# helenypzhang/Subspace-Multimodal-Learning

Hardware: AMD Instinct MI355X
Metric: bags/sec fwd+bwd, DeformCrossTransMIL N=10k x 512 (higher is better)
Workload: dtype f32

## Files before the change

subspace-multimodal-learning_amd/csrc/deform_attn.hip:

```cpp
#include "deform_common.h"
#include "cpb_regions.h"
#include "cpb_regions1d.h"

extern "C" int smml_deform_attn_nst(int N);

namespace {


constexpr int FWD_WPS = 2;
template <int PDX, bool SAVE>
__global__ __launch_bounds__(256, FWD_WPS) void deform_attn_fwd_kernel(
    const float* __restrict__ Q, const float* __restrict__ K, const float* __restrict__ V,
    const float* __restrict__ VS, const float* __restrict__ GQ, CpbParams cp, float* __restrict__ O,
    float* __restrict__ LSE, float* __restrict__ LT, unsigned short* __restrict__ MK, int N, int J, int H, int G, int NST,
    float scale, DropCfg dc_in) {
  constexpr int PD = PosCfg<PDX>::PD;
  constexpr bool RAW = PosCfg<PDX>::RAW;
  const DropCfg dc = drop_resolve(dc_in);
  __shared__ __attribute__((aligned(16))) _Float16 Kp[2][KT * FRLD];
  __shared__ __attribute__((aligned(16))) _Float16 Vp[2][KT * FTLD];
  __shared__ __attribute__((aligned(16))) _Float16 Qp[WAVES][2][QT * FRLD];
  __shared__ float vsl[KT][2];
  __shared__ float biasT[WAVES][KT][QT];

// ... 133 lines not shown
    wave_lds_fence();

    float tmax = -INFINITY;
#pragma unroll
    for (int r = 0; r < 16; ++r) {
      const int key = acc_row(r, hf);
      const float sv = (key < nk) ? s[r] + biasT[wave][key][c] : -INFINITY;
      s[r] = sv;
      tmax = fmaxf(tmax, sv);
    }
    unsigned keepbits = 0xFFFFu;
    if (dc.thresh) {
      const unsigned long long base2 = ((unsigned long long)(b * H + h) * N + qi) * ((J + 1) >> 1) + (j0 >> 1);
      keepbits = 0u;
#pragma unroll
      for (int r = 0; r < 16; r += 2) keepbits |= drop_keep2(dc, base2 + (acc_row(r, hf) >> 1)) << r;
    }
    if (SAVE) {
      if (dc.thresh) {
        tmax = -INFINITY;
#pragma unroll
        for (int r = 0; r < 16; ++r) {
          if (acc_row(r, hf) < nk) s[r] = stash_keep(s[r], (keepbits >> r) & 1u);
          tmax = fmaxf(tmax, s[r]);
        }
      }
#pragma unroll
      for (int r = 0; r < 16; ++r) {
        const int key = acc_row(r, hf);
        if (key < nk) LTb[(size_t)(j0 + key) * 32 + c] = s[r];
      }
    }
    tmax = xhalf_max(tmax);
    const float m_new = fmaxf(m_run, tmax);
    const float alpha = sexp(m_run - m_new);
    float psum = 0.f;
#pragma unroll
    for (int r = 0; r < 16; ++r) {
      const float p = sexp(s[r] - m_new);
      psum += p;
      s[r] = p;
    }
    if (dc.thresh) {
#pragma unroll
      for (int r = 0; r < 16; ++r) s[r] *= ((keepbits >> r) & 1u) ? dc.keep_scale : 0.f;
    }
    l_run = l_run * alpha + psum;
    m_run = m_new;
#pragma unroll
    for (int r = 0; r < 16; ++r) { oacc0[r] *= alpha; oacc1[r] *= alpha; }

#pragma unroll
    for (int kb = 0; kb < 2; ++kb) {
      float p8[8];
#pragma unroll
      for (int j = 0; j < 8; ++j) p8[j] = s[8 * kb + j];
      half8 ph, pl;
      split8(p8, ph, pl);
      const int ro = (16 * kb + 4 * hf + trq) * FTLD + trc;
      const half8 vh0 = lds_frag_tr_h(&Vp[0][ro], &Vp[0][ro + 8 * FTLD]), vl0 = lds_frag_tr_h(&Vp[1][ro], &Vp[1][ro + 8 * FTLD]);
      const half8 vh1 = lds_frag_tr_h(&Vp[0][ro + 32], &Vp[0][ro + 32 + 8 * FTLD]), vl1 = lds_frag_tr_h(&Vp[1][ro + 32], &Vp[1][ro + 32 + 8 * FTLD]);
      oacc0 = mfma16(vl0, ph, oacc0); oacc0 = mfma16(vh0, pl, oacc0); oacc0 = mfma16(vh0, ph, oacc0);
      oacc1 = mfma16(vl1, ph, oacc1); oacc1 = mfma16(vh1, pl, oacc1); oacc1 = mfma16(vh1, ph, oacc1);
    }
    wave_lds_fence();
  }

  l_run = xhalf_sum(l_run);
  const float inv = 1.f / l_run;
  if (qvalid) {
    float* op = O + ((size_t)b * N + qi) * HD + h * DH;
#pragma unroll
    for (int rg = 0; rg < 4; ++rg) {
      const int d = 8 * rg + 4 * hf;
      *reinterpret_cast<float4*>(op + d) = make_float4(oacc0[4 * rg] * inv, oacc0[4 * rg + 1] * inv,
                                                       oacc0[4 * rg + 2] * inv, oacc0[4 * rg + 3] * inv);
      *reinterpret_cast<float4*>(op + 32 + d) = make_float4(oacc1[4 * rg] * inv, oacc1[4 * rg + 1] * inv,
                                                            oacc1[4 * rg + 2] * inv, oacc1[4 * rg + 3] * inv);
    }
    if (hf == 0) LSE[(size_t)(b * H + h) * N + qi] = m_run + logf(l_run);
  }
}


__global__ __launch_bounds__(256, 2) void deform_attn_bwd_dq_kernel(
    const float* __restrict__ K, const float* __restrict__ V, const float* __restrict__ O,
    const float* __restrict__ dO, const float* __restrict__ LSE, const float* __restrict__ LT,
    float* __restrict__ dLT, float* __restrict__ dQ, float* __restrict__ RHO, unsigned* __restrict__ AMAX, int N, int J, int H, int NST,
    float scale, DropCfg dc_in) {
  const DropCfg dc = drop_resolve(dc_in);
  __shared__ __attribute__((aligned(16))) __bf16 Vp[2][3][KT * VBLD];
  __shared__ __attribute__((aligned(16))) __bf16 Kp[2][3][KT * KBLD];

  const int tid = threadIdx.x, wave = tid >> 6, lane = tid & 63, c = lane & 31, hf = lane >> 5;
  const int b = blockIdx.z, h = blockIdx.y;
  const int q0 = blockIdx.x * (QT * WAVES) + wave * QT;
  const int HD = H * DH;
  const bool qvalid = (q0 + c) < N;
  const int qi = qvalid ? (q0 + c) : (N - 1);

  bf16x8 doh[4], dom[4], dol[4];
  float delta = 0.f;
  {
    const size_t off = ((size_t)b * N + qi) * HD + h * DH + hf * 8;
#pragma unroll
    for (int kb = 0; kb < 4; ++kb) {
      const float4 t0 = *reinterpret_cast<const float4*>(dO + off + 16 * kb), t1 = *reinterpret_cast<const float4*>(dO + off + 16 * kb + 4);
      const float4 u0 = *reinterpret_cast<const float4*>(O + off + 16 * kb), u1 = *reinterpret_cast<const float4*>(O + off + 16 * kb + 4);
      delta += t0.x * u0.x + t0.y * u0.y + t0.z * u0.z + t0.w * u0.w + t1.x * u1.x + t1.y * u1.y + t1.z * u1.z + t1.w * u1.w;
      const float x8[8] = {t0.x, t0.y, t0.z, t0.w, t1.x, t1.y, t1.z, t1.w};
      split8_bf3(x8, doh[kb], dom[kb], dol[kb]);
    }
  }
  delta = xhalf_sum(delta);
  const float nl = prob_bias(LSE[(size_t)(b * H + h) * N + qi]);

  floatx16 dq0 = {0}, dq1 = {0};
  float amax = 0.f;
  float rho = 0.f;
  const float* Kb = K + (size_t)b * J * HD + h * DH;
  const float* Vb = V + (size_t)b * J * HD + h * DH;
  const float* LTb = LT + ((size_t)(b * H + h) * NST + q0) * J;
  float* dLTb = dLT + ((size_t)(b * H + h) * NST + q0) * J;

  const int skey = tid >> 4, sd4 = (tid & 15) * 4;
  const int trq = (lane & 15) >> 2, trc = 16 * ((lane >> 4) & 1) + 4 * (lane & 3);
  float4 kreg[2], vreg[2];
  float lt[16];
  auto fetch = [&](int j0, float4 (&kr)[2], float4 (&vr)[2], float (&l)[16]) {
#pragma unroll
    for (int i = 0; i < 2; ++i) {
      const int key = j0 + skey + 16 * i;
      kr[i] = make_float4(0.f, 0.f, 0.f, 0.f); vr[i] = kr[i];
      if (key < J) {
        kr[i] = *reinterpret_cast<const float4*>(Kb + (size_t)key * HD + sd4);
        vr[i] = *reinterpret_cast<const float4*>(Vb + (size_t)key * HD + sd4);
      }
    }
#pragma unroll
    for (int r = 0; r < 16; ++r) {
      const int key = min(j0 + acc_row(r, hf), J - 1);
      l[r] = LTb[(size_t)key * 32 + c];
    }
  };
  fetch(0, kreg, vreg, lt);

  const int ntiles = (J + KT - 1) / KT;
  for (int kt = 0; kt < ntiles; ++kt) {
    const int j0 = kt * KT, buf = kt & 1;
    const int nk = min(KT, J - j0);
#pragma unroll
    for (int i = 0; i < 2; ++i) {
      const int key = skey + 16 * i;
      uint2v hh, mm, ll;
      split4_bf3(vreg[i], hh, mm, ll);
      *reinterpret_cast<uint2v*>(&Vp[buf][0][key * VBLD + sd4]) = hh;
      *reinterpret_cast<uint2v*>(&Vp[buf][1][key * VBLD + sd4]) = mm;
      *reinterpret_cast<uint2v*>(&Vp[buf][2][key * VBLD + sd4]) = ll;
      split4_bf3(kreg[i], hh, mm, ll);
      *reinterpret_cast<uint2v*>(&Kp[buf][0][key * KBLD + sd4]) = hh;
      *reinterpret_cast<uint2v*>(&Kp[buf][1][key * KBLD + sd4]) = mm;
    }
    __syncthreads();
    float ltc[16];
#pragma unroll
    for (int r = 0; r < 16; ++r) ltc[r] = lt[r];
    if (kt + 1 < ntiles) fetch(j0 + KT, kreg, vreg, lt);

    floatx16 dp = {0};
#pragma unroll
    for (int kb = 0; kb < 4; ++kb) {
      const int o = c * VBLD + 16 * kb + 8 * hf;
      const bf16x8 vh = *reinterpret_cast<const bf16x8*>(&Vp[buf][0][o]);
      const bf16x8 vm = *reinterpret_cast<const bf16x8*>(&Vp[buf][1][o]);
      const bf16x8 vl = *reinterpret_cast<const bf16x8*>(&Vp[buf][2][o]);
      dp = bwd_prod<3>(vh, vm, vl, doh[kb], dom[kb], dol[kb], dp);
    }

    float ds[16];
    if (nk == KT && q0 + QT <= N) {
#pragma unroll
      for (int r = 0; r < 16; ++r) {
        const float p = prob_of(ltc[r], nl);
        float dpr = dp[r];
        if (dc.thresh) dpr *= stashed_factor(ltc[r], dc.keep_scale);
        const float v = p * (dpr - delta);
        dLTb[(size_t)(j0 + acc_row(r, hf)) * 32 + c] = v;
        ds[r] = v;
        rho += v;
        amax = fmaxf(amax, fabsf(v));
      }
    } else {
#pragma unroll
      for (int r = 0; r < 16; ++r) {
        const int key = acc_row(r, hf);
        float v = 0.f;
        if (key < nk && qvalid) {
          const float p = prob_of(ltc[r], nl);
          float dpr = dp[r];
          if (dc.thresh) dpr *= stashed_factor(ltc[r], dc.keep_scale);
          v = p * (dpr - delta);
          dLTb[(size_t)(j0 + key) * 32 + c] = v;
        }
        ds[r] = v;
        rho += v;
        amax = fmaxf(amax, fabsf(v));
      }
    }
#pragma unroll
    for (int kb = 0; kb < 2; ++kb) {
      float x8[8];
#pragma unroll
      for (int jx = 0; jx < 8; ++jx) x8[jx] = ds[8 * kb + jx];
      bf16x8 sh, sm, sl;
      split8_bf3(x8, sh, sm, sl);
      const int ro = (16 * kb + 4 * hf + trq) * KBLD + trc;
#pragma unroll
      for (int db = 0; db < 2; ++db) {
        const bf16x8 kh = lds_frag_tr(&Kp[buf][0][ro + 32 * db], &Kp[buf][0][ro + 32 * db + 8 * KBLD]);
        const bf16x8 km = lds_frag_tr(&Kp[buf][1][ro + 32 * db], &Kp[buf][1][ro + 32 * db + 8 * KBLD]);
        if (db == 0) dq0 = bwd_prod<2>(kh, km, km, sh, sm, sm, dq0);
        else dq1 = bwd_prod<2>(kh, km, km, sh, sm, sm, dq1);
      }
    }
  }
  rho = xhalf_sum(rho);
  if (qvalid && hf == 0) RHO[(size_t)(b * H + h) * N + qi] = rho;
  if (AMAX) {
    amax = wave_max_all(amax);
    if (lane == 0 && amax > 0.f) atomicMax(AMAX, __float_as_uint(amax));
  }
  if (qvalid) {
    float* qp = dQ + ((size_t)b * N + qi) * HD + h * DH;
#pragma unroll
    for (int rg = 0; rg < 4; ++rg) {
      const int d = 8 * rg + 4 * hf;
      *reinterpret_cast<float4*>(qp + d) = make_float4(dq0[4 * rg] * scale, dq0[4 * rg + 1] * scale,
                                                       dq0[4 * rg + 2] * scale, dq0[4 * rg + 3] * scale);
      *reinterpret_cast<float4*>(qp + 32 + d) = make_float4(dq1[4 * rg] * scale, dq1[4 * rg + 1] * scale,
                                                            dq1[4 * rg + 2] * scale, dq1[4 * rg + 3] * scale);
    }
  }
}


__global__ __launch_bounds__(256, 2) void deform_attn_bwd_dkv_kernel(
    const float* __restrict__ Q, const float* __restrict__ dO, const float* __restrict__ LSE,
    const float* __restrict__ LT, const float* __restrict__ dLT, float* __restrict__ dKp,
    float* __restrict__ dVp, int N, int J, int H, int NST, int nkg, int tiles_per_part, int nparts, int Bn, DropCfg dc_in) {
  const DropCfg dc = drop_resolve(dc_in);
  __shared__ __attribute__((aligned(16))) __bf16 Qp[2][3][QT * QBLD];
  __shared__ __attribute__((aligned(16))) __bf16 dOp[2][3][QT * QBLD];
  __shared__ __attribute__((aligned(16))) float nls[2][QT];
  const int tid = threadIdx.x, wave = tid >> 6, lane = tid & 63, c = lane & 31, hf = lane >> 5;
  const int nslices = nparts * H * Bn;
  const int chunk = blockIdx.x / (8 * nkg), rem = blockIdx.x - chunk * (8 * nkg);
  const int kg = rem >> 3, slice = chunk * 8 + (rem & 7);
  if (slice >= nslices) return;
  const int part = slice % nparts, h = (slice / nparts) % H, b = slice / (nparts * H);
  const int j0 = kg * DKV_KEYS + wave * KT;
  const int HD = H * DH;
  const int nk = min(KT, J - j0);
  const bool kvalid = c < nk;
  const int key = min(j0 + c, J - 1);
  const float* LTk = LT + (size_t)(b * H + h) * NST * J + (size_t)key * 32;
  const float* dLTk = dLT + (size_t)(b * H + h) * NST * J + (size_t)key * 32;
  const float* LSEb = LSE + (size_t)(b * H + h) * N;

  const int nqt = (N + QT - 1) / QT;
  const int qt_begin = part * tiles_per_part, qt_end = min(qt_begin + tiles_per_part, nqt);

  const int srow = tid >> 4, sd4 = (tid & 15) * 4;
  const int trq = (lane & 15) >> 2, trc = 16 * ((lane >> 4) & 1) + 4 * (lane & 3);
  float4 qreg[2], doreg[2], ltr[4], dlr[4];
  float lsereg = 0.f;
#pragma unroll
  for (int i = 0; i < 4; ++i) { ltr[i] = make_float4(0.f, 0.f, 0.f, 0.f); dlr[i] = ltr[i]; qreg[i >> 1] = ltr[i]; doreg[i >> 1] = ltr[i]; }
  auto fetch = [&](int q0) {
#pragma unroll
    for (int i = 0; i < 2; ++i) {
      const int qrow = min(q0 + srow + 16 * i, N - 1);
      const size_t off = ((size_t)b * N + qrow) * HD + h * DH + sd4;
      qreg[i] = *reinterpret_cast<const float4*>(Q + off);
      doreg[i] = *reinterpret_cast<const float4*>(dO + off);
    }
#pragma unroll
    for (int rg = 0; rg < 4; ++rg) {
      const size_t qq = (size_t)q0 * J + 8 * rg + 4 * hf;
      ltr[rg] = *reinterpret_cast<const float4*>(LTk + qq);
      dlr[rg] = *reinterpret_cast<const float4*>(dLTk + qq);
    }
    if (tid < QT) lsereg = LSEb[min(q0 + tid, N - 1)];
  };

  floatx16 dk0 = {0}, dk1 = {0}, dv0 = {0}, dv1 = {0};
  if (qt_begin < qt_end) fetch(qt_begin * QT);
  for (int qt = qt_begin; qt < qt_end; ++qt) {
    const int q0 = qt * QT, buf = (qt - qt_begin) & 1;
#pragma unroll
    for (int i = 0; i < 2; ++i) {
      const int o = (srow + 16 * i) * QBLD + sd4;
      uint2v hh, mm, ll;
      split4_bf3(qreg[i], hh, mm, ll);
      *reinterpret_cast<uint2v*>(&Qp[buf][0][o]) = hh;
      *reinterpret_cast<uint2v*>(&Qp[buf][1][o]) = mm;
      split4_bf3(doreg[i], hh, mm, ll);
      *reinterpret_cast<uint2v*>(&dOp[buf][0][o]) = hh;
      *reinterpret_cast<uint2v*>(&dOp[buf][1][o]) = mm;
    }
    if (tid < QT) nls[buf][tid] = prob_bias(lsereg);
    __syncthreads();
    float lv[16], dsv[16], ls[16];
#pragma unroll
    for (int rg = 0; rg < 4; ++rg) {
      lv[4 * rg + 0] = ltr[rg].x; lv[4 * rg + 1] = ltr[rg].y; lv[4 * rg + 2] = ltr[rg].z; lv[4 * rg + 3] = ltr[rg].w;
      dsv[4 * rg + 0] = dlr[rg].x; dsv[4 * rg + 1] = dlr[rg].y; dsv[4 * rg + 2] = dlr[rg].z; dsv[4 * rg + 3] = dlr[rg].w;
      const float4 t = *reinterpret_cast<const float4*>(&nls[buf][8 * rg + 4 * hf]);
      ls[4 * rg + 0] = t.x; ls[4 * rg + 1] = t.y; ls[4 * rg + 2] = t.z; ls[4 * rg + 3] = t.w;
    }
    if (qt + 1 < qt_end) fetch(q0 + QT);
    if (nk > 0) {
      float p[16], ds[16];
      if (nk == KT && q0 + QT <= N) {
#pragma unroll
        for (int r = 0; r < 16; ++r) {
          float pv = prob_of(lv[r], ls[r]);
          if (dc.thresh) pv *= stashed_factor(lv[r], dc.keep_scale);
          p[r] = pv; ds[r] = dsv[r];
        }
      } else {
#pragma unroll
        for (int r = 0; r < 16; ++r) {
          const int qq = q0 + acc_row(r, hf);
          const bool ok = kvalid && qq < N;
          float pv = ok ? prob_of(lv[r], ls[r]) : 0.f;
          if (dc.thresh && ok) pv *= stashed_factor(lv[r], dc.keep_scale);
          p[r] = pv;
          ds[r] = ok ? dsv[r] : 0.f;
        }
      }
#pragma unroll
      for (int kb = 0; kb < 2; ++kb) {
        float x8[8], y8[8];
#pragma unroll
        for (int jx = 0; jx < 8; ++jx) { x8[jx] = p[8 * kb + jx]; y8[jx] = ds[8 * kb + jx]; }
        bf16x8 ph, pm, pl, sh, sm, sl;
        split8_bf3(x8, ph, pm, pl);
        split8_bf3(y8, sh, sm, sl);
        const int ro = (16 * kb + 4 * hf + trq) * QBLD + trc;
#pragma unroll
        for (int db = 0; db < 2; ++db) {
          const int o = ro + 32 * db;
          const bf16x8 ah = lds_frag_tr(&dOp[buf][0][o], &dOp[buf][0][o + 8 * QBLD]);
          const bf16x8 am = lds_frag_tr(&dOp[buf][1][o], &dOp[buf][1][o + 8 * QBLD]);
          const bf16x8 qh = lds_frag_tr(&Qp[buf][0][o], &Qp[buf][0][o + 8 * QBLD]);
          const bf16x8 qm = lds_frag_tr(&Qp[buf][1][o], &Qp[buf][1][o + 8 * QBLD]);
          if (db == 0) { dv0 = bwd_prod<2>(ah, am, am, ph, pm, pm, dv0); dk0 = bwd_prod<2>(qh, qm, qm, sh, sm, sm, dk0); }
          else { dv1 = bwd_prod<2>(ah, am, am, ph, pm, pm, dv1); dk1 = bwd_prod<2>(qh, qm, qm, sh, sm, sm, dk1); }
        }
      }
    }
  }
  if (kvalid) {
    const size_t off = (((size_t)part * Bn + b) * J + (j0 + c)) * HD + h * DH;
    float* kp = dKp + off;
    float* vp = dVp + off;
#pragma unroll
    for (int rg = 0; rg < 4; ++rg) {
      const int d = 8 * rg + 4 * hf;
      *reinterpret_cast<float4*>(kp + d) = make_float4(dk0[4 * rg], dk0[4 * rg + 1], dk0[4 * rg + 2], dk0[4 * rg + 3]);
      *reinterpret_cast<float4*>(kp + 32 + d) = make_float4(dk1[4 * rg], dk1[4 * rg + 1], dk1[4 * rg + 2], dk1[4 * rg + 3]);
      *reinterpret_cast<float4*>(vp + d) = make_float4(dv0[4 * rg], dv0[4 * rg + 1], dv0[4 * rg + 2], dv0[4 * rg + 3]);
      *reinterpret_cast<float4*>(vp + 32 + d) = make_float4(dv1[4 * rg], dv1[4 * rg + 1], dv1[4 * rg + 2], dv1[4 * rg + 3]);
    }
  }
}


template <int PDX>
__global__ __launch_bounds__(256, 2) void cpb_bwd_kernel(
    const float* __restrict__ dLT, const unsigned short* __restrict__ MK, const float* __restrict__ LT,
    const float* __restrict__ LSE, const float* __restrict__ RHO, const float* __restrict__ VS,
    const float* __restrict__ GQ, CpbParams cp, float* __restrict__ slab, float* __restrict__ dvs_slab, int N, int J, int H,
    int G, int NST) {
  constexpr int PD = PosCfg<PDX>::PD;
  constexpr bool RAW = PosCfg<PDX>::RAW;
  extern __shared__ __attribute__((aligned(16))) float smem[];
  const int tid = threadIdx.x, wave = tid >> 6, lane = tid & 63, c = lane & 31, hf = lane >> 5;
  const int b = blockIdx.z, h = blockIdx.y;
  const int q0 = blockIdx.x * (QT * WAVES) + wave * QT;
  const int o = H / G, g = h / o, oi = h - g * o;
  const bool qvalid = (q0 + c) < N;
  const int qi = qvalid ? (q0 + c) : (N - 1);

  float* tab = smem;
  float* wbase = smem + CPB2_TAB;
  float* xq = wbase + wave * CPB2_WAVE_LDS;
  float2* stg = reinterpret_cast<float2*>(xq + CPB_XQ);
  const int wg = (blockIdx.z * gridDim.y + blockIdx.y) * gridDim.x + blockIdx.x;
  float2* dvs_row = reinterpret_cast<float2*>(dvs_slab) + (size_t)(wg * WAVES + wave) * J;
  if (tid < 32) {
    const int ch = acc_row(tid & 15, tid >> 4);
    tab[(tid >> 4) * 32 + (tid & 15)] = cp.w1[ch * PD];
    tab[(tid >> 4) * 32 + 16 + (tid & 15)] = (PD == 2) ? cp.w1[ch * PD + 1] : 0.f;
  }
  const float* tabh = tab + hf * 32;

  const float gq0 = GQ[(size_t)qi * PD];
  const float gq1 = (PD == 2) ? GQ[(size_t)qi * PD + 1] : 0.f;

  bf16x8 a1q, a1t;
  floatx16 b1acc;
  {
    const float wx = cp.w1[c * PD], wy = (PD == 2) ? cp.w1[c * PD + 1] : 0.f, bb = cp.b1[c];
    const __bf16 xh = (__bf16)wx; const float xr = wx - (float)xh; const __bf16 xm = (__bf16)xr;
    const __bf16 xl = (__bf16)(xr - (float)xm);
    const __bf16 yh = (__bf16)wy; const float yr = wy - (float)yh; const __bf16 ym = (__bf16)yr;
    const __bf16 yl = (__bf16)(yr - (float)ym);
    const __bf16 bh_ = (__bf16)bb; const float br = bb - (float)bh_; const __bf16 bm = (__bf16)br;
    const __bf16 bl_ = (__bf16)(br - (float)bm);
    const __bf16 z = (__bf16)0.f;
    a1q = cpb_l1_weights_q(wx, wy, hf);
    if (hf == 0) a1t = (bf16x8){xh, yh, xh, yh, xh, yh, bh_, bm};
    else a1t = (bf16x8){xm, ym, xm, ym, xl, yl, bl_, z};
#pragma unroll
    for (int s16 = 0; s16 < 16; ++s16) b1acc[s16] = cp.b1[acc_row(s16, hf)];
  }
  const float b2c = cp.b2[c];
  const float w3c = cp.w3[oi * CH + c];

  half8 w2th[2], w2tm[2], w2tl[2];
  half8 idb[2];
  float unlift2;
  {
    float amax = 0.f;
#pragma unroll
    for (int s = 0; s < 16; ++s) { const int ch = acc_row(s, hf); amax = fmaxf(amax, fabsf(cp.w2[ch * CH + c] * cp.w3[oi * CH + ch])); }
    const float lift2 = pow2_lift(wave_max_all(amax), 256.f, -8.f, 24.f);
    unlift2 = 1.f / lift2;
#pragma unroll
    for (int kb = 0; kb < 2; ++kb) {
      float t[8];
#pragma unroll
      for (int j = 0; j < 8; ++j) {
        const int ch = acc_row(8 * kb + j, hf);
        const float sc = (j & 1) ? 0.5f : 128.f;
        t[j] = cp.w2[ch * CH + c] * cp.w3[oi * CH + ch] * sc * lift2;
        idb[kb][j] = (ch == c) ? (_Float16)sc : (_Float16)0.0f;
      }
      split8_3(t, w2th[kb], w2tm[kb], w2tl[kb]);
    }
  }

  float big;
  asm("s_mov_b32 %0, 0x71800000" : "=s"(big));
  floatx16 e = {0};
  float2v aw1x[8], aw1y[8], ab1[8];
#pragma unroll
  for (int p = 0; p < 8; ++p) { aw1x[p] = (float2v){0.f, 0.f}; aw1y[p] = aw1x[p]; ab1[p] = aw1x[p]; }
  float ab3 = 0.f;
  float2v s2 = {0.f, 0.f};

  const float* VSb = VS + (size_t)(b * G + g) * J * PD;
  const float* dLTb = dLT + ((size_t)(b * H + h) * NST + q0) * J;
  __syncthreads();
// ... 147 lines not shown
    }
  }
#pragma unroll
  for (int r = 0; r < 16; ++r) {
    const int row = acc_row(r, hf);
    red[row * CH + c] = 0.5f * e[r] * cp.w3[oi * CH + row];
    float v;
    v = 0.5f * e[r] * cp.w2[row * CH + c];
#pragma unroll
    for (int off = 16; off > 0; off >>= 1) v += __shfl_xor(v, off);
    if (c == 0) red[1024 + 64 + 32 + 32 + row] += v;
    v = ab1[r >> 1][r & 1];
#pragma unroll
    for (int off = 16; off > 0; off >>= 1) v += __shfl_xor(v, off);
    if (c == 0) red[1024 + 64 + row] = v;
    v = aw1x[r >> 1][r & 1];
#pragma unroll
    for (int off = 16; off > 0; off >>= 1) v += __shfl_xor(v, off);
    if (c == 0) red[1024 + row * 2] = v;
    v = aw1y[r >> 1][r & 1];
#pragma unroll
    for (int off = 16; off > 0; off >>= 1) v += __shfl_xor(v, off);
    if (c == 0) red[1024 + row * 2 + 1] = v;
  }
  {
    float v = wave_sum(ab3);
    if (lane == 0) red[1024 + 64 + 32 + 32 + 32] = v;
  }
  __syncthreads();
  float* sl = slab + (size_t)wg * CPB_SLAB;
  const float* r0 = wbase + WAVES * CPB2_WAVE_LDS;
  for (int i = tid; i < CPB_SLAB; i += 256)
    sl[i] = (r0[i] + r0[CPB_SLAB + i]) + (r0[2 * CPB_SLAB + i] + r0[3 * CPB_SLAB + i]);
}


template <int PDX>
__global__ __launch_bounds__(256) void relu1_masks_kernel(const float* __restrict__ VS, const float* __restrict__ GQ,
                                                          const float* __restrict__ w1, const float* __restrict__ b1,
                                                          unsigned short* __restrict__ MK, int N, int J, int G, int NST) {
  constexpr int PD = PosCfg<PDX>::PD;
  constexpr bool RAW = PosCfg<PDX>::RAW;
  const int tid = threadIdx.x, wave = tid >> 6, lane = tid & 63, c = lane & 31, hf = lane >> 5;
  const int b = blockIdx.z, g = blockIdx.y;
  const int q0 = blockIdx.x * (QT * WAVES) + wave * QT;
  const int qi = min(q0 + c, N - 1);
  const float gq0 = GQ[(size_t)qi * PD];
  const float gq1 = (PD == 2) ? GQ[(size_t)qi * PD + 1] : 0.f;
  const bf16x8 a1 = cpb_l1_weights_q(w1[c * PD], (PD == 2) ? w1[c * PD + 1] : 0.f, hf);
  floatx16 b1acc;
#pragma unroll
  for (int s = 0; s < 16; ++s) b1acc[s] = b1[acc_row(s, hf)];
  const float* VSb = VS + (size_t)(b * G + g) * J * PD;
  unsigned short* MKb = MK + ((size_t)(b * G + g) * J * 2 + hf) * NST;
  for (int j = 0; j < J; ++j) {
    const float p0 = pos_of<RAW>(gq0 - VSb[(size_t)j * PD]);
    const float p1 = (PD == 2) ? slog1p(gq1 - VSb[(size_t)j * PD + 1]) : 0.f;
    const floatx16 xacc = cpb_layer1_q(a1, cpb_split_pos(p0, p1), hf, b1acc);
    unsigned m = 0;
#pragma unroll
    for (int r = 0; r < 16; ++r) m |= (xacc[r] > 0.f) ? (1u << ((13 + r) & 15)) : 0u;
    MKb[(size_t)j * 2 * NST + q0 + c] = (unsigned short)m;
  }
}


__global__ void drop_mask_kernel(float* __restrict__ mask, unsigned long long total, int J, DropCfg dc_in) {
  const DropCfg dc = drop_resolve(dc_in);
  const unsigned long long i = (unsigned long long)blockIdx.x * blockDim.x + threadIdx.x;
  if (i >= total) return;
  const unsigned long long row = i / (unsigned long long)J;
  const int j = (int)(i - row * (unsigned long long)J);
  mask[i] = (dc.thresh == 0 || ((drop_keep2(dc, row * (unsigned long long)((J + 1) >> 1) + (j >> 1)) >> (j & 1)) & 1u)) ? 1.f : 0.f;
}

template <int PDX> auto fwd_kernel(bool save) { return save ? deform_attn_fwd_kernel<PDX, true> : deform_attn_fwd_kernel<PDX, false>; }

int bwd_dq_dkv(const char* fn, const float* q, const float* k, const float* v, const float* out, const float* dout, const float* lse,
                      const float* logits_t, float* dlogits_t, float* dq, float* dk, float* dv, float* wsf, unsigned* amax, int B, int N, int J,
                      int H, float scale, DropCfg dc, hipStream_t st) {
  const BwdWorkspace wsl = bwd_workspace(B, N, J, H);
  const int nst = smml_deform_attn_nst(N);
  const int qtiles = (N + QT * WAVES - 1) / (QT * WAVES);
  hipLaunchKernelGGL(deform_attn_bwd_dq_kernel, dim3(qtiles, H, B), dim3(256), 0, st, k, v, out, dout, lse, logits_t, dlogits_t, dq, wsf + wsl.rho,
                     amax, N, J, H, nst, scale, dc);
  if (int rc = launch_check(fn, "dq")) return rc;
  const DkvGrid g = dkv_grid(B, N, J, H);
  hipLaunchKernelGGL(deform_attn_bwd_dkv_kernel, g.grid, dim3(256), 0, st, q, dout, lse, logits_t, dlogits_t, wsf + wsl.dkp, wsf + wsl.dvp, N, J, H,
                     nst, g.nkg, g.tpp, g.parts, B, dc);
  if (int rc = launch_check(fn, "dkv")) return rc;
  return dkv_reduce_launch(fn, wsf, wsl, dk, dv, B, J, H, g.parts, scale, st);
}

}

extern "C" {

int smml_deform_attn_nst(int N) { return (N <= 0 || N > SMML_MAX_QUERIES) ? 0 : (N + QT * WAVES - 1) / (QT * WAVES) * (QT * WAVES); }

int smml_deform_attn_dropout_mask_f32(float* mask, int B, int N, int J, int H, float dropout_p, unsigned long long dropout_seed,
                                      void* stream, const SmmlDeformOpts* opts) {
  SMML_REQUIRE(mask && deform_dims_ok(B, N, J, H) && dropout_p >= 0.f && dropout_p < 1.f,
               "smml_deform_attn_dropout_mask_f32: bad argument");
  const unsigned long long total = (unsigned long long)B * H * N * J;
  hipLaunchKernelGGL(drop_mask_kernel, dim3((unsigned)((total + 255) / 256)), dim3(256), 0, (hipStream_t)stream, mask, total, J,
                     make_drop(dropout_p, dropout_seed, opts));
  SMML_LAUNCH_CHECK("smml_deform_attn_dropout_mask_f32");
  return SMML_OK;
}

int smml_deform_attn_relu1_masks(const float* vs, const float* gq, const float* w1, const float* b1, unsigned short* masks, int B,
                                 int N, int J, int G, int posdim, void* stream, const SmmlDeformOpts* opts) {
  SMML_REQUIRE(vs && gq && w1 && b1 && masks && deform_dims_ok(B, N, J, G) && (posdim == 1 || posdim == 2),
               "smml_deform_attn_relu1_masks: bad argument");
  dim3 grid((N + QT * WAVES - 1) / (QT * WAVES), G, B), block(256);
  const int nst = smml_deform_attn_nst(N);
  if (posdim == 2)
    hipLaunchKernelGGL(relu1_masks_kernel<2>, grid, block, 0, (hipStream_t)stream, vs, gq, w1, b1, masks, N, J, G, nst);
  else if (pdx_of(posdim, opts) == 3)
    hipLaunchKernelGGL(relu1_masks_kernel<3>, grid, block, 0, (hipStream_t)stream, vs, gq, w1, b1, masks, N, J, G, nst);
  else
    hipLaunchKernelGGL(relu1_masks_kernel<1>, grid, block, 0, (hipStream_t)stream, vs, gq, w1, b1, masks, N, J, G, nst);
  SMML_LAUNCH_CHECK("smml_deform_attn_relu1_masks");
  return SMML_OK;
}

size_t smml_deform_attn_bwd_workspace_bytes(int B, int N, int J, int H) {
  if (!deform_dims_ok(B, N, J, H)) return 0;
  return bwd_workspace(B, N, J, H).total * sizeof(float);
}

int smml_deform_attn_fwd_f32(const float* q, const float* k, const float* v, const float* vs, const float* gq,
                             const float* w1, const float* b1, const float* w2, const float* b2,
                             const float* w3, const float* b3, float* out, float* lse, float* logits_t,
                             unsigned short* relu_masks, int B, int N, int J, int H, int G, int posdim, float scale,
                             float dropout_p, unsigned long long dropout_seed, void* ev_start, void* ev_stop, void* stream, const SmmlDeformOpts* opts) {
  static const char* fn = "smml_deform_attn_fwd_f32";
  int rc = check_common(fn, B, N, J, H, G, posdim);
  if (!rc) rc = check_dropout(fn, dropout_p);
  if (rc) return rc;
  SMML_REQUIRE(q && k && v && vs && gq && w1 && b1 && w2 && b2 && w3 && b3 && out && lse, "%s: null pointer", fn);
  if ((rc = check_saved(fn, logits_t, relu_masks, "logits_t", "relu_masks"))) return rc;
  const DropCfg dc = make_drop(dropout_p, dropout_seed, opts);
  CpbParams cp{w1, b1, w2, b2, w3, b3};
  const int pdx = pdx_of(posdim, opts);
  const bool save = relu_masks != nullptr;
  const auto kern = pdx == 2 ? fwd_kernel<2>(save) : pdx == 3 ? fwd_kernel<3>(save) : fwd_kernel<1>(save);
  hipStream_t st = (hipStream_t)stream;
  if (ev_start) (void)hipEventRecord((hipEvent_t)ev_start, st);
  hipLaunchKernelGGL(kern, dim3((N + QT * WAVES - 1) / (QT * WAVES), H, B), dim3(256), 0, st, q, k, v, vs, gq, cp, out, lse, logits_t, relu_masks,
                     N, J, H, G, smml_deform_attn_nst(N), scale, dc);
  if (ev_stop) (void)hipEventRecord((hipEvent_t)ev_stop, st);
  SMML_LAUNCH_CHECK(fn);
  return SMML_OK;
}

int smml_deform_attn_bwd_f32(const float* q, const float* k, const float* v, const float* vs, const float* gq,
                             const float* w1, const float* b1, const float* w2, const float* b2,
                             const float* w3, const float* b3, const float* out, const float* dout,
                             const float* lse, const float* logits_t, const unsigned short* relu_masks,
                             float* dlogits_t, float* dq, float* dk,
                             float* dv, float* dvs, float* dw1, float* db1, float* dw2, float* db2, float* dw3,
                             float* db3, void* workspace, size_t workspace_bytes, int B, int N, int J, int H,
                             int G, int posdim, float scale, float dropout_p, unsigned long long dropout_seed,
                             void* ev_start, void* ev_stop, void* stream, const SmmlDeformOpts* opts) {
  static const char* fn = "smml_deform_attn_bwd_f32";
  int rc = check_common(fn, B, N, J, H, G, posdim);
  if (!rc) rc = check_dropout(fn, dropout_p);
  if (rc) return rc;
  SMML_REQUIRE(q && k && v && vs && gq && w1 && b1 && w2 && b2 && w3 && b3 && out && dout && lse && logits_t &&
                   relu_masks && dlogits_t && dq && dk && dv && dvs && dw1 && db1 && dw2 && db2 && dw3 && db3 && workspace,
               "%s: null pointer", fn);
  if ((rc = check_workspace(fn, workspace, workspace_bytes, smml_deform_attn_bwd_workspace_bytes(B, N, J, H), 16))) return rc;
  const DropCfg dc = make_drop(dropout_p, dropout_seed, opts);
  CpbParams cp{w1, b1, w2, b2, w3, b3};
  hipStream_t st = (hipStream_t)stream;
  const int qtiles = (N + QT * WAVES - 1) / (QT * WAVES);
  const BwdWorkspace wsl = bwd_workspace(B, N, J, H);
  float* wsf = reinterpret_cast<float*>(workspace);
  if ((rc = bwd_dq_dkv(fn, q, k, v, out, dout, lse, logits_t, dlogits_t, dq, dk, dv, wsf, nullptr, B, N, J, H, scale, dc, st))) return rc;
  const int pdx = pdx_of(posdim, opts);
  const auto kern = pdx == 2 ? cpb_bwd_kernel<2> : pdx == 3 ? cpb_bwd_kernel<3> : cpb_bwd_kernel<1>;
  const size_t lds = ((size_t)CPB2_TAB + WAVES * CPB2_WAVE_LDS + WAVES * CPB_SLAB) * sizeof(float);
  if (ev_start) (void)hipEventRecord((hipEvent_t)ev_start, st);
  hipLaunchKernelGGL(kern, dim3(qtiles, H, B), dim3(256), lds, st, dlogits_t, relu_masks, logits_t, lse, wsf + wsl.rho, vs, gq, cp, wsf + wsl.slab,
                     wsf + wsl.dvs, N, J, H, G, smml_deform_attn_nst(N));
  if (ev_stop) (void)hipEventRecord((hipEvent_t)ev_stop, st);
  if ((rc = launch_check(fn, "cpb"))) return rc;
  return cpb_reduce_launch(fn, wsf, wsl, dvs, dw1, db1, dw2, db2, dw3, db3, B, J, H, G, qtiles, posdim, st);
}


}

static int regions_build(const char* fn, const float* w1, const float* b1, const float* w2, const float* b2, const float* w3, const float* b3,
                         int outputs, float pmax, void* tables, size_t tables_bytes, void* stream) {
  SMML_REQUIRE(w1 && b1 && w2 && b2 && w3 && b3 && tables, "%s: null pointer", fn);
  SMML_REQUIRE(outputs == 1 || outputs == 2, "%s: outputs (heads per offset group) must be 1 or 2 (got %d)", fn, outputs);
  SMML_REQUIRE(pmax > 0.f && pmax < 16.f, "%s: pmax must be in (0, 16) (got %g)", fn, (double)pmax);
  SMML_REQUIRE(tables_bytes >= region_layout().total, "%s: table buffer too small (%zu < %zu)", fn, tables_bytes, region_layout().total);
  SMML_REQUIRE((reinterpret_cast<size_t>(tables) & 255) == 0, "%s: table buffer must be 256-byte aligned", fn);
  region_build_launch(CpbParams{w1, b1, w2, b2, w3, b3}, pmax, tables, (hipStream_t)stream, outputs);
  SMML_LAUNCH_CHECK(fn);
  return SMML_OK;
}
static size_t region_bwd_bytes(int B, int N, int J, int H, int G) {
  if (!deform_dims_ok(B, N, J, H) || J > RG_MAX_KEYS || G <= 0 || H % G || H / G > RG_HPG) return 0;
  return region_bwd_plan(B, N, J, H, H / G).total;
}

template <bool MH>
static int region_fwd_f32(const char* fn, const float* q, const float* k, const float* v, const float* vs, const float* gq, const float* w1,
                          const float* b1, const float* w2, const float* b2, const float* w3, const float* b3, const void* tables, float* out,
                          float* lse, float* logits_t, unsigned short* region_ids, int B, int N, int J, int H, int G, float scale, float dropout_p,
                          unsigned long long dropout_seed, void* ev_start, void* ev_stop, void* stream, const SmmlDeformOpts* opts) {
  int rc = check_region(fn, B, N, J, H, G);
  if (!rc) rc = check_dropout(fn, dropout_p);
  if (rc) return rc;
  SMML_REQUIRE(q && k && v && vs && gq && w1 && b1 && w2 && b2 && w3 && b3 && tables && out && lse, "%s: null pointer", fn);
  if ((rc = check_saved(fn, logits_t, region_ids, "logits_t", "region_ids"))) return rc;
  const DropCfg dc = make_drop(dropout_p, dropout_seed, opts);
  CpbParams cp{w1, b1, w2, b2, w3, b3};
  const RegionView rv = region_view(const_cast<void*>(tables));
  const auto kern = region_ids ? deform_region_fwd_kernel<true, float, MH> : deform_region_fwd_kernel<false, float, MH>;
  hipStream_t st = (hipStream_t)stream;
  if (ev_start) (void)hipEventRecord((hipEvent_t)ev_start, st);
  hipLaunchKernelGGL(kern, dim3((N + QT * WAVES - 1) / (QT * WAVES), H, B), dim3(256), 0, st, q, k, v, vs, gq, cp, rv, out, lse, logits_t, region_ids,
                     N, J, H, smml_deform_attn_nst(N), scale, dc, region_lcap(opts), G);
  if (ev_stop) (void)hipEventRecord((hipEvent_t)ev_stop, st);
  SMML_LAUNCH_CHECK(fn);
  return SMML_OK;
}

template <bool MH>
static int region_bwd_f32(const char* fn, const float* q, const float* k, const float* v, const float* vs, const float* gq, const float* w1,
                          const float* b1, const float* w2, const float* b2, const float* w3, const float* b3, const void* tables, const float* out,
                          const float* dout, const float* lse, const float* logits_t, const unsigned short* region_ids, float* dlogits_t, float* dq,
                          float* dk, float* dv, float* dvs, float* dw1, float* db1, float* dw2, float* db2, float* dw3, float* db3, void* workspace,
                          size_t workspace_bytes, int B, int N, int J, int H, int G, float scale, float dropout_p, unsigned long long dropout_seed,
                          void* ev_start, void* ev_stop, void* stream, const SmmlDeformOpts* opts) {
  int rc = check_region(fn, B, N, J, H, G);
  if (!rc) rc = check_dropout(fn, dropout_p);
  if (rc) return rc;
  SMML_REQUIRE(q && k && v && vs && gq && w1 && b1 && w2 && b2 && w3 && b3 && tables && out && dout && lse && logits_t && region_ids &&
                   dlogits_t && dq && dk && dv && dvs && dw1 && db1 && dw2 && db2 && dw3 && db3 && workspace,
               "%s: null pointer", fn);
  const RegionBwdPlan pl = region_bwd_plan(B, N, J, H, H / G);
  if ((rc = check_region_workspace(fn, workspace, workspace_bytes, pl, J))) return rc;
  const DropCfg dc = make_drop(dropout_p, dropout_seed, opts);
  hipStream_t st = (hipStream_t)stream;
  char* wsb = reinterpret_cast<char*>(workspace);
  (void)hipMemsetAsync(wsb + pl.amax, 0, pl.dvs - pl.amax, st);
  rc = bwd_dq_dkv(fn, q, k, v, out, dout, lse, logits_t, dlogits_t, dq, dk, dv, reinterpret_cast<float*>(workspace),
                  reinterpret_cast<unsigned*>(wsb + pl.amax), B, N, J, H, scale, dc, st);
  if (rc) return rc;
  return region_bias_bwd_launch<float, MH>(fn, dlogits_t, region_ids, vs, gq, CpbParams{w1, b1, w2, b2, w3, b3}, tables, wsb, pl, B, N, J, H, G,
                                           smml_deform_attn_nst(N), region_lcap(opts), dvs, dw1, db1, dw2, db2, dw3, db3, ev_start, ev_stop, st);
}

extern "C" {

size_t smml_cpb_regions_bytes(void) { return region_layout().total; }

int smml_cpb_regions_build(const float* w1, const float* b1, const float* w2, const float* b2, const float* w3, const float* b3,
                           float pmax, void* tables, size_t tables_bytes, void* stream) {
  return regions_build("smml_cpb_regions_build", w1, b1, w2, b2, w3, b3, 1, pmax, tables, tables_bytes, stream);
}

// ... 126 lines not shown
```

subspace-multimodal-learning_amd/csrc/deform_common.h:

```cpp
#pragma once
#include "smml_common.h"

namespace {

__device__ __forceinline__ float slog1p(float d) {
  return copysignf(__builtin_amdgcn_logf(fabsf(d) + 1.0f) * 0.6931471805599453f, d);
}
__device__ __forceinline__ float sexp(float x) { return __expf(x); }
__device__ __forceinline__ float srcp(float x) { return __builtin_amdgcn_rcpf(x); }
__device__ __forceinline__ float relu2(float x) { return x + __builtin_fabsf(x); }

template <int PDX> struct PosCfg {
  static constexpr int PD = (PDX == 3) ? 1 : PDX;
  static constexpr bool RAW = (PDX == 3);
};
template <bool RAW> __device__ __forceinline__ float pos_of(float d) { return RAW ? d : slog1p(d); }
template <bool RAW> __device__ __forceinline__ float dpos_of(float d, float big) {
  return RAW ? 1.f : srcp(fabsf(d) + 1.f) * fminf(fmaxf(fabsf(d) * big, 0.f), 1.f);
}
constexpr int DH = 64;
constexpr int CH = 32;
constexpr int QT = 32;
constexpr int WAVES = 4;
constexpr int KT = 32;
// ... 187 lines not shown
  const long long out = t >> 2;
  const bool ok = out < (long long)Bn * G * J;
  float2 s = make_float2(0.f, 0.f);
  if (ok) {
    const int j = (int)(out % J);
    const int bg = (int)(out / J), b = bg / G, g = bg - b * G, o = H / G;
    for (int oi = 0; oi < o; ++oi) {
      const float2* p = rows + ((size_t)((b * H + g * o + oi) * qtiles) * WAVES + w) * J + j;
#pragma unroll 8
      for (int x = 0; x < qtiles; ++x) {
        const float2 v = p[(size_t)x * WAVES * J];
        s.x += v.x; s.y += v.y;
      }
    }
  }
  s.x += __shfl_xor(s.x, 1); s.y += __shfl_xor(s.y, 1);
  s.x += __shfl_xor(s.x, 2); s.y += __shfl_xor(s.y, 2);
  if (ok && w == 0) {
    dVS[out * PD] = s.x;
    if (PD == 2) dVS[out * PD + 1] = s.y;
  }
}

constexpr int CPB_RED_CHUNKS = 64;
__global__ void cpb_partial_kernel(const float* __restrict__ slab, int nwg, int o, int wg_per_head, int H, int chunk,
                                   float* __restrict__ part_out) {
  const int k = blockIdx.x * 64 + (threadIdx.x & 63);
  const int part = threadIdx.x >> 6, nparts = blockDim.x >> 6;
  const int w0 = blockIdx.y * chunk, w1 = min(w0 + chunk, nwg);
  __shared__ float acc[4][64][2];
  float s0 = 0.f, s1 = 0.f;
  if (k < CPB_SLAB) {
    for (int w = w0 + part; w < w1; w += nparts) {
      const int hh = (w / wg_per_head) % H;
      const int oi = hh % o;
      const float v = slab[(size_t)w * CPB_SLAB + k];
      if (oi == 0) s0 += v; else if (oi == 1) s1 += v;
    }
  }
  acc[part][threadIdx.x & 63][0] = s0;
  acc[part][threadIdx.x & 63][1] = s1;
  __syncthreads();
  if (part == 0 && k < CPB_SLAB) {
    float t0 = 0.f, t1 = 0.f;
    for (int p = 0; p < nparts; ++p) { t0 += acc[p][threadIdx.x][0]; t1 += acc[p][threadIdx.x][1]; }
    part_out[((size_t)blockIdx.y * CPB_SLAB + k) * 2 + 0] = t0;
    part_out[((size_t)blockIdx.y * CPB_SLAB + k) * 2 + 1] = t1;
  }
}
__global__ void cpb_final_kernel(const float* __restrict__ part_in, int nchunks, int o, float* __restrict__ dW1,
                                 float* __restrict__ db1, float* __restrict__ dW2, float* __restrict__ db2,
                                 float* __restrict__ dW3, float* __restrict__ db3, int PD) {
  const int k = blockIdx.x * blockDim.x + threadIdx.x;
  if (k >= CPB_SLAB) return;
  float t0 = 0.f, t1 = 0.f;
  for (int p = 0; p < nchunks; ++p) {
    t0 += part_in[((size_t)p * CPB_SLAB + k) * 2 + 0];
    t1 += part_in[((size_t)p * CPB_SLAB + k) * 2 + 1];
  }
  if (k < 1024) dW2[k] = t0 + t1;
  else if (k < 1024 + 64) {
    const int ch = (k - 1024) >> 1, comp = (k - 1024) & 1;
    if (comp < PD) dW1[ch * PD + comp] = t0 + t1;
  } else if (k < 1024 + 96) db1[k - 1088] = t0 + t1;
  else if (k < 1024 + 128) db2[k - 1120] = t0 + t1;
  else if (k < 1024 + 160) {
    dW3[k - 1152] = t0;
    if (o > 1) dW3[CH + k - 1152] = t1;
  } else if (k == 1024 + 160) {
    db3[0] = t0;
    if (o > 1) db3[1] = t1;
  }
}

static int dkv_parts(int B, int N, int J, int H) {
  const int nkg = (J + DKV_KEYS - 1) / DKV_KEYS, nqt = (N + QT - 1) / QT;
  const long base = (long)nkg * H * B;
  long parts = (1280 + base / 2) / base;
  if (parts < 1) parts = 1;
  if (parts > 16) parts = 16;
  if (parts > nqt) parts = nqt;
  return (int)parts;
}
struct BwdWorkspace {
  size_t slab, partial, dkp, dvp, rho, dvs, total;
};
static BwdWorkspace bwd_workspace(int B, int N, int J, int H) {
  BwdWorkspace w;
  const size_t nwg = (size_t)B * H * ((N + QT * WAVES - 1) / (QT * WAVES));
  const size_t kv = (size_t)dkv_parts(B, N, J, H) * B * J * H * DH;
  w.slab = 0;
  w.partial = nwg * CPB_SLAB;
  w.dkp = (w.partial + (size_t)CPB_RED_CHUNKS * CPB_SLAB * 2 + 3) & ~(size_t)3;
  w.dvp = w.dkp + kv;
  w.rho = w.dvp + kv;
  w.dvs = w.rho + (((size_t)B * H * N + 3) & ~(size_t)3);
  w.total = w.dvs + nwg * WAVES * (size_t)J * 2;
  return w;
}

constexpr int SMML_MAX_QUERIES = 1 << 26, SMML_MAX_KEYS = 1 << 22;
bool deform_dims_ok(int B, int N, int J, int H) {
  return B > 0 && N > 0 && J > 0 && H > 0 && B <= 65535 && H <= 65535 && N <= SMML_MAX_QUERIES && J <= SMML_MAX_KEYS;
}
int pdx_of(int posdim, const SmmlDeformOpts* opts) { return posdim == 2 ? 2 : ((opts && opts->raw_distance) ? 3 : 1); }
DropCfg make_drop(float p, unsigned long long seed, const SmmlDeformOpts* opts) {
  DropCfg dc;
  dc.seed = seed;
  dc.seed_dev = opts ? opts->seed_offset : nullptr;
  dc.thresh = (p > 0.f) ? (unsigned)fmax(1.0, (double)p * 65536.0) : 0u;
  dc.keep_scale = (p > 0.f) ? (float)(65536.0 / (65536.0 - (double)dc.thresh)) : 1.0f;
  return dc;
}

int check_common(const char* fn, int B, int N, int J, int H, int G, int posdim) {
  SMML_REQUIRE(B > 0 && N > 0 && J > 0 && H > 0 && G > 0, "%s: non-positive dimension", fn);
  SMML_REQUIRE(H % G == 0, "%s: heads (%d) must be divisible by offset groups (%d)", fn, H, G);
  SMML_REQUIRE(H / G <= 2, "%s: at most 2 heads per offset group are supported (got %d)", fn, H / G);
  SMML_REQUIRE(posdim == 1 || posdim == 2, "%s: posdim must be 1 or 2 (got %d)", fn, posdim);
  SMML_REQUIRE(deform_dims_ok(B, N, J, H), "%s: B, H <= 65535, N <= 2^26, J <= 2^22 (got B %d N %d J %d H %d)", fn, B, N, J, H);
  return SMML_OK;
}
int check_dropout(const char* fn, float p) {
  SMML_REQUIRE(p >= 0.f && p < 1.f, "%s: dropout_p must be in [0, 1)", fn);
  return SMML_OK;
}
int check_saved(const char* fn, const void* scores, const void* ids, const char* scores_name, const char* ids_name) {
  SMML_REQUIRE((scores == nullptr) == (ids == nullptr), "%s: %s and %s are saved together (training) or not at all", fn, scores_name, ids_name);
  return SMML_OK;
}
int check_workspace(const char* fn, const void* ws, size_t bytes, size_t need, size_t align) {
  SMML_REQUIRE(bytes >= need, "%s: workspace too small (%zu < %zu)", fn, bytes, need);
  SMML_REQUIRE((reinterpret_cast<size_t>(ws) & (align - 1)) == 0, "%s: workspace must be %zu-byte aligned", fn, align);
  return SMML_OK;
}
int launch_check(const char* fn, const char* pass) {
  const hipError_t e = hipGetLastError();
  if (e == hipSuccess) return SMML_OK;
  smml_set_error("%s/%s: launch failed: %s", fn, pass, hipGetErrorString(e));
  return SMML_ERR_HIP;
}

struct DkvGrid {
  int nkg, parts, tpp;
  dim3 grid;
};
DkvGrid dkv_grid(int B, int N, int J, int H) {
  DkvGrid g;
  g.nkg = (J + DKV_KEYS - 1) / DKV_KEYS;
  g.parts = dkv_parts(B, N, J, H);
  g.tpp = ((N + QT - 1) / QT + g.parts - 1) / g.parts;
  const int nslices = g.parts * H * B;
  g.grid = dim3(((nslices + 7) / 8) * 8 * g.nkg);
  return g;
}
int dkv_reduce_launch(const char* fn, const float* wsf, const BwdWorkspace& wsl, float* dk, float* dv, int B, int J, int H, int parts,
                      float scale, hipStream_t st) {
  const size_t n4 = (size_t)B * J * H * DH / 4;
  hipLaunchKernelGGL(dkv_reduce_kernel, dim3((unsigned)((n4 + 255) / 256)), dim3(256), 0, st, reinterpret_cast<const float4*>(wsf + wsl.dkp),
                     reinterpret_cast<const float4*>(wsf + wsl.dvp), reinterpret_cast<float4*>(dk), reinterpret_cast<float4*>(dv), n4, parts, scale);
  return launch_check(fn, "dkv_reduce");
}

int cpb_reduce_launch(const char* fn, float* wsf, const BwdWorkspace& wsl, float* dvs, float* dw1, float* db1, float* dw2, float* db2,
                      float* dw3, float* db3, int B, int J, int H, int G, int qtiles, int posdim, hipStream_t st) {
  const int nwg = qtiles * H * B;
  const long long threads = (long long)B * G * J * 4;
  hipLaunchKernelGGL(dvs_reduce_kernel, dim3((unsigned)((threads + 255) / 256)), dim3(256), 0, st, reinterpret_cast<const float2*>(wsf + wsl.dvs),
                     dvs, B, G, H, qtiles, J, posdim);
  const int nchunks = min(CPB_RED_CHUNKS, nwg), chunk = (nwg + nchunks - 1) / nchunks;
  hipLaunchKernelGGL(cpb_partial_kernel, dim3((CPB_SLAB + 63) / 64, nchunks), dim3(256), 0, st, wsf + wsl.slab, nwg, H / G, qtiles, H, chunk,
                     wsf + wsl.partial);
  hipLaunchKernelGGL(cpb_final_kernel, dim3((CPB_SLAB + 255) / 256), dim3(256), 0, st, wsf + wsl.partial, nchunks, H / G, dw1, db1, dw2, db2, dw3,
                     db3, posdim);
  return launch_check(fn, "reduce");
}

}
```

Measured before the change: 1231.

## Presplit K/V into bf16 planes once per backward pass for dQ kernel

A new kv_split_kernel converts K and V once into packed bf16 hi/mid/lo planes in workspace, tiled by KT. The dQ kernel then copies these planes straight into LDS instead of re-splitting the fp32 K/V tile in every query workgroup, and drops the unused third K plane from LDS. The unused RHO row-sum and its workspace slot are removed, the LT/dLT addressing is simplified, and the dKV kernel's Q/dO LDS buffers shrink from three planes to two. In exchange there is an extra kernel launch, and each tile read is 5 bf16 planes rather than two fp32 arrays, which is slightly more bytes per element.

Result: no change. 1235 (median of 6 runs) (+0.3%).

```diff
diff --git a/subspace-multimodal-learning_amd/csrc/deform_attn.hip b/subspace-multimodal-learning_amd/csrc/deform_attn.hip
--- a/subspace-multimodal-learning_amd/csrc/deform_attn.hip
+++ b/subspace-multimodal-learning_amd/csrc/deform_attn.hip
@@ -239,15 +239,38 @@
   }
 }
 
+__global__ __launch_bounds__(256) void kv_split_kernel(const float* __restrict__ K, const float* __restrict__ V, uint4v* __restrict__ P, int J,
+                                                       int H) {
+  const int tid = threadIdx.x, row = tid >> 3, d8 = (tid & 7) * 8;
+  const int b = blockIdx.z, h = blockIdx.y, key = blockIdx.x * KT + row;
+  float4 k0 = make_float4(0.f, 0.f, 0.f, 0.f), k1 = k0, v0 = k0, v1 = k0;
+  if (key < J) {
+    const size_t off = ((size_t)b * J + key) * (H * DH) + h * DH + d8;
+    k0 = *reinterpret_cast<const float4*>(K + off); k1 = *reinterpret_cast<const float4*>(K + off + 4);
+    v0 = *reinterpret_cast<const float4*>(V + off); v1 = *reinterpret_cast<const float4*>(V + off + 4);
+  }
+  uint2v h0, m0, l0, h1, m1, l1;
+  uint4v* out = P + ((size_t)(b * H + h) * gridDim.x + blockIdx.x) * KV_TILE_U4 + tid;
+  split4_bf3(v0, h0, m0, l0);
+  split4_bf3(v1, h1, m1, l1);
+  out[0 * KV_PLANE_U4] = (uint4v){h0[0], h0[1], h1[0], h1[1]};
+  out[1 * KV_PLANE_U4] = (uint4v){m0[0], m0[1], m1[0], m1[1]};
+  out[2 * KV_PLANE_U4] = (uint4v){l0[0], l0[1], l1[0], l1[1]};
+  split4_bf3(k0, h0, m0, l0);
+  split4_bf3(k1, h1, m1, l1);
+  out[3 * KV_PLANE_U4] = (uint4v){h0[0], h0[1], h1[0], h1[1]};
+  out[4 * KV_PLANE_U4] = (uint4v){m0[0], m0[1], m1[0], m1[1]};
+}
+
 
 __global__ __launch_bounds__(256, 2) void deform_attn_bwd_dq_kernel(
-    const float* __restrict__ K, const float* __restrict__ V, const float* __restrict__ O,
+    const uint4v* __restrict__ KVP, const float* __restrict__ O,
     const float* __restrict__ dO, const float* __restrict__ LSE, const float* __restrict__ LT,
-    float* __restrict__ dLT, float* __restrict__ dQ, float* __restrict__ RHO, unsigned* __restrict__ AMAX, int N, int J, int H, int NST,
+    float* __restrict__ dLT, float* __restrict__ dQ, unsigned* __restrict__ AMAX, int N, int J, int H, int NST,
     float scale, DropCfg dc_in) {
   const DropCfg dc = drop_resolve(dc_in);
   __shared__ __attribute__((aligned(16))) __bf16 Vp[2][3][KT * VBLD];
-  __shared__ __attribute__((aligned(16))) __bf16 Kp[2][3][KT * KBLD];
+  __shared__ __attribute__((aligned(16))) __bf16 Kp[2][2][KT * KBLD];
 
   const int tid = threadIdx.x, wave = tid >> 6, lane = tid & 63, c = lane & 31, hf = lane >> 5;
   const int b = blockIdx.z, h = blockIdx.y;
@@ -274,55 +297,47 @@
 
   floatx16 dq0 = {0}, dq1 = {0};
   float amax = 0.f;
-  float rho = 0.f;
-  const float* Kb = K + (size_t)b * J * HD + h * DH;
-  const float* Vb = V + (size_t)b * J * HD + h * DH;
-  const float* LTb = LT + ((size_t)(b * H + h) * NST + q0) * J;
-  float* dLTb = dLT + ((size_t)(b * H + h) * NST + q0) * J;
-
-  const int skey = tid >> 4, sd4 = (tid & 15) * 4;
+  const int ntiles = (J + KT - 1) / KT;
+  const uint4v* KVb = KVP + (size_t)(b * H + h) * ntiles * KV_TILE_U4 + tid;
+  const size_t lto = ((size_t)(b * H + h) * NST + q0) * J + 4 * hf * 32 + c;
+  const float* LTb = LT + lto;
+  float* dLTb = dLT + lto;
+
+  const int skey = tid >> 3, sd8 = (tid & 7) * 8;
   const int trq = (lane & 15) >> 2, trc = 16 * ((lane >> 4) & 1) + 4 * (lane & 3);
-  float4 kreg[2], vreg[2];
+  uint4v pl[KV_PLANES];
   float lt[16];
-  auto fetch = [&](int j0, float4 (&kr)[2], float4 (&vr)[2], float (&l)[16]) {
-#pragma unroll
-    for (int i = 0; i < 2; ++i) {
-      const int key = j0 + skey + 16 * i;
-      kr[i] = make_float4(0.f, 0.f, 0.f, 0.f); vr[i] = kr[i];
-      if (key < J) {
-        kr[i] = *reinterpret_cast<const float4*>(Kb + (size_t)key * HD + sd4);
-        vr[i] = *reinterpret_cast<const float4*>(Vb + (size_t)key * HD + sd4);
-      }
-    }
-#pragma unroll
-    for (int r = 0; r < 16; ++r) {
-      const int key = min(j0 + acc_row(r, hf), J - 1);
-      l[r] = LTb[(size_t)key * 32 + c];
+  auto fetch = [&](int kt, uint4v (&pr)[KV_PLANES], float (&l)[16]) {
+    const uint4v* src = KVb + (size_t)kt * KV_TILE_U4;
+#pragma unroll
+    for (int i = 0; i < KV_PLANES; ++i) pr[i] = src[i * KV_PLANE_U4];
+    const int j0 = kt * KT;
+    if (j0 + KT <= J) {
+      const float* p = LTb + (size_t)j0 * 32;
+#pragma unroll
+      for (int r = 0; r < 16; ++r) l[r] = p[acc_row(r, 0) * 32];
+    } else {
+#pragma unroll
+      for (int r = 0; r < 16; ++r) {
+        const int key = min(j0 + acc_row(r, hf), J - 1);
+        l[r] = LTb[(ptrdiff_t)(key - 4 * hf) * 32];
+      }
     }
   };
-  fetch(0, kreg, vreg, lt);
-
-  const int ntiles = (J + KT - 1) / KT;
+  fetch(0, pl, lt);
+
   for (int kt = 0; kt < ntiles; ++kt) {
     const int j0 = kt * KT, buf = kt & 1;
     const int nk = min(KT, J - j0);
 #pragma unroll
-    for (int i = 0; i < 2; ++i) {
-      const int key = skey + 16 * i;
-      uint2v hh, mm, ll;
-      split4_bf3(vreg[i], hh, mm, ll);
-      *reinterpret_cast<uint2v*>(&Vp[buf][0][key * VBLD + sd4]) = hh;
-      *reinterpret_cast<uint2v*>(&Vp[buf][1][key * VBLD + sd4]) = mm;
-      *reinterpret_cast<uint2v*>(&Vp[buf][2][key * VBLD + sd4]) = ll;
-      split4_bf3(kreg[i], hh, mm, ll);
-      *reinterpret_cast<uint2v*>(&Kp[buf][0][key * KBLD + sd4]) = hh;
-      *reinterpret_cast<uint2v*>(&Kp[buf][1][key * KBLD + sd4]) = mm;
-    }
+    for (int i = 0; i < 3; ++i) *reinterpret_cast<uint4v*>(&Vp[buf][i][skey * VBLD + sd8]) = pl[i];
+#pragma unroll
+    for (int i = 0; i < 2; ++i) *reinterpret_cast<uint4v*>(&Kp[buf][i][skey * KBLD + sd8]) = pl[3 + i];
     __syncthreads();
     float ltc[16];
 #pragma unroll
     for (int r = 0; r < 16; ++r) ltc[r] = lt[r];
-    if (kt + 1 < ntiles) fetch(j0 + KT, kreg, vreg, lt);
+    if (kt + 1 < ntiles) fetch(kt + 1, pl, lt);
 
     floatx16 dp = {0};
 #pragma unroll
@@ -336,15 +351,15 @@
 
     float ds[16];
     if (nk == KT && q0 + QT <= N) {
+      float* dp0 = dLTb + (size_t)j0 * 32;
 #pragma unroll
       for (int r = 0; r < 16; ++r) {
         const float p = prob_of(ltc[r], nl);
         float dpr = dp[r];
         if (dc.thresh) dpr *= stashed_factor(ltc[r], dc.keep_scale);
         const float v = p * (dpr - delta);
-        dLTb[(size_t)(j0 + acc_row(r, hf)) * 32 + c] = v;
+        dp0[acc_row(r, 0) * 32] = v;
         ds[r] = v;
-        rho += v;
         amax = fmaxf(amax, fabsf(v));
       }
     } else {
@@ -357,10 +372,9 @@
           float dpr = dp[r];
           if (dc.thresh) dpr *= stashed_factor(ltc[r], dc.keep_scale);
           v = p * (dpr - delta);
-          dLTb[(size_t)(j0 + key) * 32 + c] = v;
+          dLTb[(size_t)(j0 + acc_row(r, 0)) * 32] = v;
         }
         ds[r] = v;
-        rho += v;
         amax = fmaxf(amax, fabsf(v));
       }
     }
@@ -381,8 +395,6 @@
       }
     }
   }
-  rho = xhalf_sum(rho);
-  if (qvalid && hf == 0) RHO[(size_t)(b * H + h) * N + qi] = rho;
   if (AMAX) {
     amax = wave_max_all(amax);
     if (lane == 0 && amax > 0.f) atomicMax(AMAX, __float_as_uint(amax));
@@ -406,8 +418,8 @@
     const float* __restrict__ LT, const float* __restrict__ dLT, float* __restrict__ dKp,
     float* __restrict__ dVp, int N, int J, int H, int NST, int nkg, int tiles_per_part, int nparts, int Bn, DropCfg dc_in) {
   const DropCfg dc = drop_resolve(dc_in);
-  __shared__ __attribute__((aligned(16))) __bf16 Qp[2][3][QT * QBLD];
-  __shared__ __attribute__((aligned(16))) __bf16 dOp[2][3][QT * QBLD];
+  __shared__ __attribute__((aligned(16))) __bf16 Qp[2][2][QT * QBLD];
+  __shared__ __attribute__((aligned(16))) __bf16 dOp[2][2][QT * QBLD];
   __shared__ __attribute__((aligned(16))) float nls[2][QT];
   const int tid = threadIdx.x, wave = tid >> 6, lane = tid & 63, c = lane & 31, hf = lane >> 5;
   const int nslices = nparts * H * Bn;
@@ -537,7 +549,7 @@
 template <int PDX>
 __global__ __launch_bounds__(256, 2) void cpb_bwd_kernel(
     const float* __restrict__ dLT, const unsigned short* __restrict__ MK, const float* __restrict__ LT,
-    const float* __restrict__ LSE, const float* __restrict__ RHO, const float* __restrict__ VS,
+    const float* __restrict__ LSE, const float* __restrict__ VS,
     const float* __restrict__ GQ, CpbParams cp, float* __restrict__ slab, float* __restrict__ dvs_slab, int N, int J, int H,
     int G, int NST) {
   constexpr int PD = PosCfg<PDX>::PD;
@@ -851,8 +863,11 @@
   const BwdWorkspace wsl = bwd_workspace(B, N, J, H);
   const int nst = smml_deform_attn_nst(N);
   const int qtiles = (N + QT * WAVES - 1) / (QT * WAVES);
-  hipLaunchKernelGGL(deform_attn_bwd_dq_kernel, dim3(qtiles, H, B), dim3(256), 0, st, k, v, out, dout, lse, logits_t, dlogits_t, dq, wsf + wsl.rho,
-                     amax, N, J, H, nst, scale, dc);
+  const uint4v* kvp = reinterpret_cast<const uint4v*>(wsf + wsl.kvp);
+  hipLaunchKernelGGL(kv_split_kernel, dim3((J + KT - 1) / KT, H, B), dim3(256), 0, st, k, v, const_cast<uint4v*>(kvp), J, H);
+  if (int rc = launch_check(fn, "kv_split")) return rc;
+  hipLaunchKernelGGL(deform_attn_bwd_dq_kernel, dim3(qtiles, H, B), dim3(256), 0, st, kvp, out, dout, lse, logits_t, dlogits_t, dq, amax, N, J, H,
+                     nst, scale, dc);
   if (int rc = launch_check(fn, "dq")) return rc;
   const DkvGrid g = dkv_grid(B, N, J, H);
   hipLaunchKernelGGL(deform_attn_bwd_dkv_kernel, g.grid, dim3(256), 0, st, q, dout, lse, logits_t, dlogits_t, wsf + wsl.dkp, wsf + wsl.dvp, N, J, H,
@@ -952,7 +967,7 @@
   const auto kern = pdx == 2 ? cpb_bwd_kernel<2> : pdx == 3 ? cpb_bwd_kernel<3> : cpb_bwd_kernel<1>;
   const size_t lds = ((size_t)CPB2_TAB + WAVES * CPB2_WAVE_LDS + WAVES * CPB_SLAB) * sizeof(float);
   if (ev_start) (void)hipEventRecord((hipEvent_t)ev_start, st);
-  hipLaunchKernelGGL(kern, dim3(qtiles, H, B), dim3(256), lds, st, dlogits_t, relu_masks, logits_t, lse, wsf + wsl.rho, vs, gq, cp, wsf + wsl.slab,
+  hipLaunchKernelGGL(kern, dim3(qtiles, H, B), dim3(256), lds, st, dlogits_t, relu_masks, logits_t, lse, vs, gq, cp, wsf + wsl.slab,
                      wsf + wsl.dvs, N, J, H, G, smml_deform_attn_nst(N));
   if (ev_stop) (void)hipEventRecord((hipEvent_t)ev_stop, st);
   if ((rc = launch_check(fn, "cpb"))) return rc;
diff --git a/subspace-multimodal-learning_amd/csrc/deform_common.h b/subspace-multimodal-learning_amd/csrc/deform_common.h
--- a/subspace-multimodal-learning_amd/csrc/deform_common.h
+++ b/subspace-multimodal-learning_amd/csrc/deform_common.h
@@ -293,8 +293,11 @@
   if (parts > nqt) parts = nqt;
   return (int)parts;
 }
+constexpr int KV_PLANES = 5;
+constexpr int KV_PLANE_U4 = KT * DH / 8;
+constexpr int KV_TILE_U4 = KV_PLANES * KV_PLANE_U4;
 struct BwdWorkspace {
-  size_t slab, partial, dkp, dvp, rho, dvs, total;
+  size_t slab, partial, dkp, dvp, kvp, dvs, total;
 };
 static BwdWorkspace bwd_workspace(int B, int N, int J, int H) {
   BwdWorkspace w;
@@ -304,8 +307,8 @@
   w.partial = nwg * CPB_SLAB;
   w.dkp = (w.partial + (size_t)CPB_RED_CHUNKS * CPB_SLAB * 2 + 3) & ~(size_t)3;
   w.dvp = w.dkp + kv;
-  w.rho = w.dvp + kv;
-  w.dvs = w.rho + (((size_t)B * H * N + 3) & ~(size_t)3);
+  w.kvp = w.dvp + kv;
+  w.dvs = w.kvp + (size_t)B * H * ((J + KT - 1) / KT) * KV_TILE_U4 * 4;
   w.total = w.dvs + nwg * WAVES * (size_t)J * 2;
   return w;
 }
```
